# HaydenFaulkner/VidDet

Hardware: AMD Instinct MI355X
Metric: frames/sec (416x416) yolo3_darknet53 fwd+bwd (higher is better)
Workload: dtype f32; 1 GPU; yolo3_darknet53_coco training, batch 64/GPU, 416x416, fp32, fwd+bwd+SGD-momentum (BASELINE configs[2]; the reference trains with SGD, not Adam); classes=80, global_batch=64, parallelism=dp1, hip_graph=False

## Files before the change

### include/viddet_hip.h

```cpp
#ifndef VIDDET_HIP_H
#define VIDDET_HIP_H

#include <stdint.h>

#ifdef __cplusplus
extern "C" {
#endif

#define VD_OK            0
#define VD_EINVAL       -1
#define VD_ELAUNCH      -2
#define VD_EWORKSPACE   -3

#define VD_MAX_TAPS 27

#define VD_EPI_AFFINE    1
#define VD_EPI_LEAKY     2
#define VD_EPI_RESIDUAL  4
#define VD_MATH_SPLIT    16
#define VD_MATH_BF16     32

#define VD_MATH_F16X2    64
#define VD_MATH_NOHALO   128
#define VD_STORE_BF16    256
#define VD_WGRAD_HALO    512
#define VD_CONV_STREAMK  1024
#define VD_CONV_PARITY4  2048
#define VD_CONV_SPLITK   4096
#define VD_SK_MAX_WG        2048
#define VD_SK_HEADER_BYTES  32768
#define VD_SK_SPLIT_CNT_OFF   4096
#define VD_SK_SPLIT_MAX_TILES 4096
#define VD_SK_TIMEOUT_TICKS 4000
#define VD_AMAX_SLOTS    32
#define VD_AMAX_STRIDE   64
#define VD_AMAX_FLOATS   (VD_AMAX_SLOTS * VD_AMAX_STRIDE)

const char* vd_last_error(void);
int vd_version(void);
#define VD_ABI_VERSION 8
int vd_abi_version(void);
int64_t vd_sizeof_desc(int which);

// ... 27 lines not shown
    const float* bs_mean;
    const float* bs_invstd;
    float*  bs_part;
    float   bs_slope;
    const float* amax_in;
    const float* amax_w;
    float*  amax_out;
    void*   sk_ws;
    int64_t sk_ws_bytes;
    int32_t par_cin;
    int32_t par_mask;
} vd_conv_desc;

int vd_conv_igemm(const vd_conv_desc* d, void* stream);
int vd_conv_igemm_streamk(const vd_conv_desc* d);
int64_t vd_conv_igemm_streamk_ws_bytes(void);
int vd_conv_igemm_mtiles(const vd_conv_desc* d);

int vd_conv_igemm_bf16(const vd_conv_desc* d, int out_f32, void* stream);
int vd_conv_igemm_bf16_streamk(const vd_conv_desc* d, int out_f32);
int vd_conv_igemm_bf16_mtiles(const vd_conv_desc* d);
int vd_pack_weight_bf16(const float* wp_f32, void* wp_bf16, int Co, int Co_pad, int Ci, int Ci_pad, int T,
                        void* stream);
int vd_stem_im2col_bf16(const float* in, void* col, int N, int H, int W, int nchw, void* stream);

typedef struct {
    const float* in;
    const float* dout;
    float*       dwp;
    int32_t N, Hi, Wi, Ci;
// ... 164 lines not shown
```

### viddet_amd/csrc/vd_conv.hip

```cpp

#include "vd_conv_igemm.h"

int vd_igemm_sk_dispatch(const vd_conv_desc& d, int tile, hipStream_t s);
int vd_igemm_sk_applies(const vd_conv_desc& d, int tile);
int vd_igemm_par_dispatch(const vd_conv_desc& d, int tile, hipStream_t s);
int vd_igemm_par_tile(int tile);
int vd_igemm_par_bm(int tile);

namespace {

int igemm_resolve_tile(const vd_conv_desc& d) {
    int tile = d.tile;
    if (tile <= 0 || tile > 8) {
        if (d.Co <= 32) tile = 7;
        else if (d.Co <= 64) tile = 6;
        else tile = 2;
    }
    return tile;
}

int igemm_tile_bm(int tile) { return (tile == 4 || tile == 5) ? 64 : 128; }

int igemm_split_resolve_tile(const vd_conv_desc& d) {
    int tile = d.tile;
    if (tile <= 0 || tile > 16) tile = d.Co <= 32 ? 9 : (d.Co <= 64 ? 3 : 1);
    return tile;
}
int igemm_split_tile_bm(int tile) { return (tile >= 13 ? 256 : (tile >= 11 ? 128 : ((tile >= 9 || ((tile - 1) & 3) == 0 || ((tile - 1) & 3) == 2) ? 256 : 128))); }

template <bool XF>
int dispatch_igemm_split(const vd_conv_desc& d, hipStream_t s) {
    if (!XF && (d.flags & VD_CONV_STREAMK) && vd_igemm_sk_dispatch(d, igemm_split_resolve_tile(d), s) == 0) return 0;
    switch (igemm_split_resolve_tile(d)) {
        case 1: return launch_igemm<4, 2, 2, 2, XF, true>(d, s);
        case 2: return launch_igemm<4, 2, 1, 2, XF, true>(d, s);
        case 3: return launch_igemm<4, 2, 2, 1, XF, true>(d, s);
        case 4: return launch_igemm<4, 2, 1, 1, XF, true>(d, s);
        case 5: return launch_igemm<4, 2, 2, 2, XF, true, true>(d, s);
        case 6: return launch_igemm<4, 2, 1, 2, XF, true, true>(d, s);
        case 7: return launch_igemm<4, 2, 2, 1, XF, true, true>(d, s);
        case 8: return launch_igemm<4, 2, 1, 1, XF, true, true>(d, s);
        case 9: return launch_igemm<8, 1, 1, 1, XF, true>(d, s);
        case 10: return launch_igemm<8, 1, 1, 1, XF, true, true>(d, s);
        case 11: return launch_igemm<2, 2, 2, 2, XF, true>(d, s);
        case 12: return launch_igemm<2, 2, 2, 2, XF, true, true>(d, s);
        case 13: return launch_igemm<4, 1, 2, 1, XF, true>(d, s);
// ... 561 lines not shown
                   d->Co == 4 * d->par_cin && d->ldo >= d->par_cin && d->ldo % 4 == 0 && (uintptr_t)d->out % 16 == 0 &&
                   (!(d->flags & VD_EPI_RESIDUAL) || (d->ldr % 4 == 0 && (uintptr_t)d->residual % 16 == 0)),
                   "vd_conv_igemm: VD_CONV_PARITY4 geometry (even output, Co = 4 par_cin, aligned rows)");
        VD_REQUIRE(!d->bs_part || (((uintptr_t)d->bs_z | (uintptr_t)d->bs_scale | (uintptr_t)d->bs_shift | (uintptr_t)d->bs_mean |
                                    (uintptr_t)d->bs_invstd) % 16 == 0), "vd_conv_igemm: VD_CONV_PARITY4 bs_* alignment");
        vd_igemm_par_dispatch(*d, vd_igemm_par_tile(d->tile), s);
        VD_CHECK_LAUNCH("vd_conv_igemm/parity4");
        return VD_OK;
    }
    if (d->in_scale) dispatch_igemm<true>(*d, s);
    else dispatch_igemm<false>(*d, s);
    VD_CHECK_LAUNCH("vd_conv_igemm");
    return VD_OK;
}

int vd_conv_igemm_streamk(const vd_conv_desc* d) {
    if (!d || !(d->flags & VD_CONV_STREAMK) || !(d->flags & VD_MATH_F16X2)) return 0;
    return vd_igemm_sk_applies(*d, igemm_split_resolve_tile(*d));
}

int64_t vd_conv_igemm_streamk_ws_bytes(void) {
    return (int64_t)VD_SK_HEADER_BYTES + (int64_t)device_cus() * 256 * 256 * 4;
}

int vd_conv_igemm_mtiles(const vd_conv_desc* d) {
    if (!d) return 0;
    const int64_t M = (int64_t)d->N * d->Hg * d->Wg;
    if (d->flags & VD_CONV_PARITY4)
        return (int)(vd_cdiv(M, vd_igemm_par_bm(vd_igemm_par_tile(d->tile))) * vd_cdiv(d->Co, 128));
    if (d->flags & (VD_MATH_SPLIT | VD_MATH_BF16 | VD_MATH_F16X2)) return (int)vd_cdiv(M, igemm_split_tile_bm(igemm_split_resolve_tile(*d)));
    return (int)vd_cdiv(M, igemm_tile_bm(igemm_resolve_tile(*d)));
}
// ... 132 lines not shown
```

### viddet_amd/csrc/vd_conv_igemm.h

```cpp
#pragma once
#include "vd_common.h"
#include "vd_wgrad_halo.h"
#include <stdlib.h>

namespace {


#ifndef VD_WG_REMAP
#define VD_WG_REMAP 1
#endif
#ifndef VD_KORDER
#define VD_KORDER 1
#endif
#ifndef VD_SETPRIO
#define VD_SETPRIO 1
#endif
#ifndef VD_PROBE
#define VD_PROBE 0
#endif
#ifndef VD_PD
#define VD_PD 3
#endif
#ifndef VD_BNT
#define VD_BNT 0
// ... 96 lines not shown
template <> struct Terms<3> { static constexpr int N = 6; static constexpr int QA[6] = {1, 2, 0, 1, 0, 0}, QB[6] = {1, 0, 2, 0, 1, 0}; };
template <> struct Terms<2> { static constexpr int N = 3; static constexpr int QA[6] = {1, 0, 0, 0, 0, 0}, QB[6] = {0, 1, 0, 0, 0, 0}; };
template <> struct Terms<1> { static constexpr int N = 1; static constexpr int QA[6] = {0, 0, 0, 0, 0, 0}, QB[6] = {0, 0, 0, 0, 0, 0}; };

__device__ __forceinline__ unsigned udiv_rcp(unsigned n, unsigned d, unsigned rcp) {
    unsigned q = d == 1u ? n : __umulhi(n, rcp);
    q -= (q * d > n) ? 1u : 0u;
    return q;
}

struct RowInfo {
    int64_t off;
    unsigned mask;
};

template <int WM, int WN, int TM, int TN, bool XF, bool SP, bool M16 = false, bool BS = false, int NPL = 3, bool HALO = false, bool SK = false,
          bool PAR = false>
__global__ __launch_bounds__(WM * WN * 64, ((!SP && WM * WN == 8) ? 4 : ((SP && WM * WN == 4) ? 2 : 1))) void k_conv_igemm(const vd_conv_desc p, const int64_t zd_in, const int64_t zd_w, const int sk_lds_flag, const int sk_timeout) {
    static_assert(NPL == 3 || ((NPL == 1 || NPL == 2) && SP), "planes");
    static_assert(!SK || (NPL == 2 && VD_KORDER && !VD_KROT && !XF), "stream-K: the fp16-split tiles, taps-innermost K order");
    static_assert(!PAR || (NPL == 2 && !HALO && !SK && VD_KORDER && !VD_KROT), "parity-fused data gradient: fp16-split tiles, generic loop");
    static_assert(NPL != 2 || !XF, "the fp16 split needs the max-abs of the operand it splits: no in-load transform");
    static_assert(!HALO || (NPL == 2 && WM * WN == 8 && WN * TN * 32 >= 64), "the halo loop exists for the 8-wave fp16-split tiles");
    constexpr int SP_ROWB = NPL * 64;
    constexpr int NTERM = Terms<NPL>::N;
    static_assert(!M16 || SP, "the 16x16x32 shape exists for the bf16 operands of the split arithmetic");
    constexpr int BM = WM * TM * 32, BN = WN * TN * 32;
    constexpr int NT = WM * WN * 64;
    constexpr int RPP = NT / 8;
    constexpr bool BHALF = BN < RPP;
    constexpr int AP = BM / RPP, BP = BHALF ? 1 : BN / RPP;
    static_assert(WM * WN == 4 || WM * WN == 8, "4 or 8 waves");
    static_assert(BM % RPP == 0 && (BHALF || BN % RPP == 0), "tile vs loader");
    static_assert(!BHALF || SP, "the half-populated weight pass exists for the split-math tiles");
    extern __shared__ __attribute__((aligned(16))) float smem[];
    float* As = smem;
    float* Bs = smem + 2 * BM * LDS_LD;
    char* As3 = reinterpret_cast<char*>(smem);
    char* Bs3 = As3 + 2 * BM * SP_ROWB;

    const int64_t M = (int64_t)p.N * p.Hg * p.Wg;
    const int ntile = (p.Co + BN - 1) / BN;
    const int Ktot = p.T * p.Ci;
    constexpr int KU = HALO ? 9 : 1;
    const int upt = p.T * (p.Ci / BK) / KU;
    int sk_nitems = 1, sk_t0 = 0, sk_nwhole = 0, sk_brem = 0, sk_erem = 0, sk_tlast = 0, sk_tfirst = 0, sk_me = 0;
    if (SK) {
        const int G = (int)gridDim.x, g = blockIdx.x & 7, j = blockIdx.x >> 3;
        const int gq = G >> 3, gr = G & 7;
        const int gs = gq + (g < gr ? 1 : 0);
        const int gbase = g * gq + (g < gr ? g : gr);
        const int64_t ntiles_all = vd_cdiv(M, BM) * ntile;
        const int tq = (int)(ntiles_all >> 3), tr = (int)(ntiles_all & 7);
        const int tg0 = g * tq + (g < tr ? g : tr), tgn = tq + (g < tr ? 1 : 0);
// ... 34 lines not shown
    const int lrow = tid >> 3;
    const int lc4 = (tid & 7) * 4;
    int lid = SK ? 0 : vd_xcd_remap(blockIdx.x, gridDim.x);
    int kb = 0, ke = upt;
    int sk_mode = 0;
    if (SK) {
        __syncthreads();
        const bool hasA = sk_erem != 0;
        if (hasA && sk_it == 0) { lid = sk_tlast; ke = sk_erem; sk_mode = 1; }
        else if (sk_it - (hasA ? 1 : 0) < sk_nwhole) lid = sk_t0 + sk_it - (hasA ? 1 : 0);
        else { lid = sk_tfirst; kb = sk_brem; sk_mode = 2; }
    }
    const int mt_all = (int)vd_cdiv(M, BM);
    const int tile_n = SK ? lid / mt_all : lid % ntile, tile_m = SK ? lid % mt_all : lid / ntile;
    RowInfo ri[AP];
    {
        int riy[AP], rix[AP], rfz[AP];
#pragma unroll
        for (int i = 0; i < AP; ++i) {
            const int64_t m = (int64_t)tile_m * BM + lrow + RPP * i;
            const unsigned mu = m < M ? (unsigned)m : 0u;
            const unsigned t = udiv_rcp(mu, (unsigned)p.Wg, rcp_w);
            const int gx = (int)(mu - t * (unsigned)p.Wg);
            const unsigned n_ = udiv_rcp(t, (unsigned)p.Hg, rcp_h);
            const int gy = (int)(t - n_ * (unsigned)p.Hg);
            const int n = (int)n_;
            riy[i] = gy * p.in_stride;
            rix[i] = gx * p.in_stride;
            rfz[i] = p.Kfr == 1 ? 0 : n % p.Kfr;
            ri[i].off = (int64_t)((n * p.Hi + riy[i]) * p.Wi + rix[i]) * p.Ci + lc4;
            ri[i].mask = 0u;
// ... 57 lines not shown
#pragma unroll
                    for (int ni = 0; ni < TN; ++ni)
#pragma unroll
                        for (int q = 0; q < 4; ++q) {
                            const f32x4 v = slot[((mi * TN + ni) * 4 + q) * NT + tid];
#pragma unroll
                            for (int e = 0; e < 4; ++e) acc[mi][ni][4 * q + e] = v[e];
                        }
            } else {
                kb = 0;
                sk_mode = 0;
            }
        }
    }

    constexpr int PD = (VD_PD > 2 && ((WM * WN == 4 && TM * TN == 4) || (M16 && TM * TN == 4))) ? 2 : VD_PD;
    f32x4 ra[PD][AP], rb[PD][BP];
    int t_tap = 0, c0 = VD_KROT ? (int)((unsigned)tile_m % (unsigned)(p.Ci / BK)) * BK : 0;
    if (SK && !HALO) {
        c0 = (kb / p.T) * BK;
        t_tap = kb - (kb / p.T) * p.T;
    }

    const int64_t tap_eo = (int64_t)((tap_dz * p.Hi + tap_dy) * p.Wi + tap_dx) * p.Ci;
    const int tap_eo_lo = (int)(tap_eo & 0xffffffffll), tap_eo_hi = (int)(tap_eo >> 32);
    auto tap_off = [&](int t) -> int64_t {
        const unsigned lo = (unsigned)__builtin_amdgcn_readlane(tap_eo_lo, t);
        const int hi = __builtin_amdgcn_readlane(tap_eo_hi, t);
        return ((int64_t)hi << 32) | (int64_t)lo;
    };
    int64_t tap_soff = tap_off(t_tap);
    auto gload = [&](f32x4 (&ra)[AP], f32x4 (&rb)[BP]) {
        const int64_t soff = tap_soff + c0;
        f32x4 sc = {0.f, 0.f, 0.f, 0.f}, sh = {0.f, 0.f, 0.f, 0.f};
        if (XF) {
            sc = *reinterpret_cast<const f32x4*>(p.in_scale + c0 + lc4);
            sh = *reinterpret_cast<const f32x4*>(p.in_shift + c0 + lc4);
        }
#pragma unroll
        for (int i = 0; i < AP; ++i) {
            const bool ok = (ri[i].mask >> t_tap) & 1u;
            const int64_t o = ri[i].off + soff;
            const int64_t sel = (ok && !(VD_PROBE & 8) && !((VD_PROBE & 32) && t_tap != 0)) ? o : zd_in;
            f32x4 v = *reinterpret_cast<const f32x4*>(p.in + sel);
            if (XF) {
#pragma unroll
                for (int e = 0; e < 4; ++e) {
// ... 430 lines not shown
                }
            }
            if (!late) hstores(u, do_store);
            __syncthreads();
        };
        int ks = 0;
        for (; ks + UNH + PD + 1 <= nks; ks += UNH) {
#pragma unroll
            for (int u = 0; u < UNH; ++u) hstep(u, true, true, true);
        }
        for (; ks < nks; ks += UNH) {
#pragma unroll
            for (int u = 0; u < UNH; ++u)
                if (ks + u < nks) hstep(u, ks + u + 1 < nks, ks + u + PD + 1 < nks, ks + u + 2 < nks);
        }
    } else {
    gload(ra[0], rb[0]);
    STAMP(2);
    lstore(0, ra[0], rb[0]);
    __syncthreads();
    STAMP(3);
    constexpr bool ld = !(VD_PROBE & 1), st = !(VD_PROBE & 2), bar = !(VD_PROBE & 4);
    constexpr int UN = (PD % 2 == 0) ? PD : 2 * PD;
    constexpr bool STAGGER = SP && (WM * WN == 8);
    const bool stag = (wave >> 2) & 1;
#pragma unroll
    for (int d = 1; d < PD; ++d)
        if (d < nks && ld) gload(ra[d], rb[d]);
    int ks = 0;
    if (nks >= PD) {
// ... 43 lines not shown
            __syncthreads();
            if (tid == 0)
                __hip_atomic_fetch_add(reinterpret_cast<unsigned*>(p.sk_ws) + sk_me, 1u, __ATOMIC_RELAXED, __HIP_MEMORY_SCOPE_AGENT);
            continue;
        }
    }
    if (NPL == 2) {
        const int de = -(sexp_a + sexp_b);
#pragma unroll
        for (int mi = 0; mi < TM; ++mi)
#pragma unroll
            for (int ni = 0; ni < TN; ++ni)
#pragma unroll
                for (int r = 0; r < 16; ++r) acc[mi][ni][r] = __builtin_ldexpf(acc[mi][ni][r], de);
    }
    const bool direct = (p.out_stride == 1 && p.out_oy == 0 && p.out_ox == 0 && p.Ho == p.Hg &&
                         p.Wo == p.Wg);
    float* stg = smem + wave * (32 * LDS_LD);
    const int erow = lane >> 3, ec4 = (lane & 7) * 4;
    const bool bstat = BS && p.bs_part != nullptr;
    float bs1[TN][4], bs2[TN][4];
#pragma unroll
    for (int ni = 0; ni < TN; ++ni)
#pragma unroll
        for (int e = 0; e < 4; ++e) bs1[ni][e] = bs2[ni][e] = 0.f;
    const bool vec_ok = (p.ldo % 4 == 0) && ((uintptr_t)p.out % 16 == 0) &&
                        (!(p.flags & VD_EPI_RESIDUAL) || ((p.ldr % 4 == 0) && ((uintptr_t)p.residual % 16 == 0)));
    const bool has_aff = p.flags & VD_EPI_AFFINE, has_leaky = p.flags & VD_EPI_LEAKY, has_res = p.flags & VD_EPI_RESIDUAL;
    bool fast = vec_ok && (p.Co % 4 == 0) && (!has_aff || (((uintptr_t)p.scale | (uintptr_t)p.shift) % 16 == 0));
    if (BS) fast = fast && (!bstat || (((uintptr_t)p.bs_z | (uintptr_t)p.bs_scale | (uintptr_t)p.bs_shift |
                                        (uintptr_t)p.bs_mean | (uintptr_t)p.bs_invstd) % 16 == 0));
    if (SK || fast) {
        constexpr int NB = TM * TN;
        f32x4 sc[TN], sh[TN], qsc[BS ? TN : 1], qsh[BS ? TN : 1], qmu[BS ? TN : 1], qis[BS ? TN : 1];
        int colv[TN];
        const f32x4 ones = {1.f, 1.f, 1.f, 1.f}, zeros = {0.f, 0.f, 0.f, 0.f};
#pragma unroll
        for (int ni = 0; ni < TN; ++ni) {
            const int col = tile_n * BN + wn * TN * 32 + ni * 32 + ec4;
            const int chn = PAR ? col % p.par_cin : col;
            colv[ni] = col < p.Co ? chn : -1;
            const int cc = col < p.Co ? chn : 0;
            sc[ni] = (has_aff && p.scale) ? *reinterpret_cast<const f32x4*>(p.scale + cc) : ones;
            sh[ni] = (has_aff && p.shift) ? *reinterpret_cast<const f32x4*>(p.shift + cc) : zeros;
            if (BS) {
                qsc[ni] = bstat ? *reinterpret_cast<const f32x4*>(p.bs_scale + cc) : zeros;
                qsh[ni] = bstat ? *reinterpret_cast<const f32x4*>(p.bs_shift + cc) : zeros;
// ... 63 lines not shown
                    amx = fmaxf(amx, fmaxf(fmaxf(fabsf(t[0]), fabsf(t[1])), fmaxf(fabsf(t[2]), fabsf(t[3]))));
                }
                if (BS && bstat) {
                    const f32x4 z = rz[BS ? (b & S1) : 0][i];
#pragma unroll
                    for (int e = 0; e < 4; ++e) {
                        const float u = z[e] * qsc[ni][e] + qsh[ni][e];
                        float g = u > 0.f ? t[e] : t[e] * p.bs_slope;
                        g = ok ? g : 0.f;
                        bs1[ni][e] += g;
                        bs2[ni][e] += g * (z[e] - qmu[ni][e]) * qis[ni][e];
                    }
                }
            }
        }
    } else if constexpr (!SK) {
#pragma unroll
    for (int ni = 0; ni < TN; ++ni) {
        const int col = tile_n * BN + wn * TN * 32 + ni * 32 + ec4;
        const int nvalid = p.Co - col;
        float sc[4] = {1.f, 1.f, 1.f, 1.f}, sh[4] = {0.f, 0.f, 0.f, 0.f};
        if (p.flags & VD_EPI_AFFINE) {
#pragma unroll
            for (int e = 0; e < 4; ++e)
                if (e < nvalid) {
                    if (p.scale) sc[e] = p.scale[col + e];
                    if (p.shift) sh[e] = p.shift[col + e];
                }
        }
        float qsc[4], qsh[4], qmu[4], qis[4];
        if (bstat) {
// ... 196 lines not shown
    }
    if (p.amax_out) vd_amax_publish(p.amax_out, amx);
    STAMP(6);
}

const float* zero_page() {
    static const float* zp = nullptr;
    if (!zp) {
        void* q = nullptr;
        if (hipGetSymbolAddress(&q, HIP_SYMBOL(g_zero_page)) != hipSuccess) q = nullptr;
        zp = (const float*)q;
    }
    return zp;
}

template <int WM, int WN, int TM, int TN, bool XF, bool SP, bool M16, bool BS, int NPL, bool HALO = false, bool SK = false, bool PAR = false>
int launch_igemm_bs(const vd_conv_desc& d, hipStream_t s);

inline int64_t halo_lds_bytes(int BM, int BN, int W) { return 2ll * (BM + 2 * (W + 1) + 2) * 128 + 3ll * BN * 128; }

inline bool halo_ok(const vd_conv_desc& d, int BM, int BN) {
    if (!(d.flags & VD_MATH_F16X2) || (d.flags & VD_MATH_NOHALO) || d.in_scale || d.T != 9 || d.in_stride != 1 || d.Kfr != 1 ||
        d.Hg != d.Hi || d.Wg != d.Wi || BN < 64)
        return false;
    for (int t = 0; t < 9; ++t)
        if (d.dy[t] < -1 || d.dy[t] > 1 || d.dx[t] < -1 || d.dx[t] > 1 || d.dz[t] != 0) return false;
    return BM + 2 * (d.Wi + 1) <= 8 * 64 && halo_lds_bytes(BM, BN, d.Wi) <= 160 * 1024;
}

template <int WM, int WN, int TM, int TN, bool XF, bool SP = false, bool M16 = false>
int launch_igemm(const vd_conv_desc& d, hipStream_t s) {
    if (SP && (d.flags & VD_MATH_BF16)) {
        if (d.bs_part) return launch_igemm_bs<WM, WN, TM, TN, false, SP, M16, true, SP ? 1 : 3>(d, s);
        return launch_igemm_bs<WM, WN, TM, TN, false, SP, M16, false, SP ? 1 : 3>(d, s);
    }
    if (SP && (d.flags & VD_MATH_F16X2)) {
        constexpr bool HT_ = SP && WM * WN == 8 && WN * TN * 32 >= 64;
        if (HT_ && halo_ok(d, WM * TM * 32, WN * TN * 32)) {
            if (d.bs_part) return launch_igemm_bs<WM, WN, TM, TN, false, SP, M16, true, SP ? 2 : 3, HT_>(d, s);
            return launch_igemm_bs<WM, WN, TM, TN, false, SP, M16, false, SP ? 2 : 3, HT_>(d, s);
        }
        if (d.bs_part) return launch_igemm_bs<WM, WN, TM, TN, false, SP, M16, true, SP ? 2 : 3>(d, s);
// ... 16 lines not shown
inline int streamk_grid(const vd_conv_desc& d, int BM, int BN, int wg_per_cu) {
    if (!(d.flags & VD_CONV_STREAMK) || !d.sk_ws) return 0;
    auto al16 = [](const void* q) { return (uintptr_t)q % 16 == 0; };
    if (d.ldo % 4 || d.Co % 4 || !al16(d.out) || ((d.flags & VD_EPI_RESIDUAL) && (d.ldr % 4 || !al16(d.residual))) ||
        ((d.flags & VD_EPI_AFFINE) && (!al16(d.scale) || !al16(d.shift))) ||
        (d.bs_part && !(al16(d.bs_z) && al16(d.bs_scale) && al16(d.bs_shift) && al16(d.bs_mean) && al16(d.bs_invstd))))
        return 0;
    const int64_t ntiles = vd_cdiv((int64_t)d.N * d.Hg * d.Wg, BM) * vd_cdiv(d.Co, BN);
    const int G = device_cus() * wg_per_cu;
    if (G > VD_SK_MAX_WG - 2 || G < 8 || (ntiles >> 3) < (G + 7) / 8) return 0;
    if (ntiles <= G + G / 16) return 0;
    if (d.sk_ws_bytes < (int64_t)VD_SK_HEADER_BYTES + (int64_t)G * BM * BN * 4) return 0;
    return G;
}

template <int WM, int WN, int TM, int TN, bool XF, bool SP, bool M16, bool BS, int NPL, bool HALO, bool SK, bool PAR>
int launch_igemm_bs(const vd_conv_desc& d, hipStream_t s) {
    constexpr int BM = WM * TM * 32, BN = WN * TN * 32;
    constexpr int lds0 = SP ? 2 * (BM + BN) * NPL * 64 : 2 * (BM + BN) * LDS_LD * (int)sizeof(float);
    constexpr int lds_epi = WM * WN * 32 * LDS_LD * 4 > WM * BN * 2 * 4 ? WM * WN * 32 * LDS_LD * 4 : WM * BN * 2 * 4;
    constexpr int lds_fixed = lds0 > lds_epi ? lds0 : lds_epi;
    static_assert(lds_fixed + (SK ? 16 : 0) <= 160 * 1024, "LDS budget");
    int lds = lds_fixed;
    if (HALO) {
        const int64_t hb = halo_lds_bytes(BM, BN, d.Wi);
        lds = hb > lds_epi ? (int)hb : lds_epi;
    }
    int64_t nblk = vd_cdiv((int64_t)d.N * d.Hg * d.Wg, BM) * vd_cdiv(d.Co, BN);
    int sk_flag_off = 0;
    if (SK) {
        const int G = streamk_grid(d, BM, BN, (SP && WM * WN == 4) ? 2 : 1);
        lds = (lds + 15) & ~15;
        if (G == 0 || lds + 16 > 160 * 1024) return 1;
        sk_flag_off = lds;
        lds += 16;
        nblk = G;
    }
    static bool attr_done = false;
    auto kfn = k_conv_igemm<WM, WN, TM, TN, XF, SP, M16, BS, NPL, HALO, SK, PAR>;
    if (!attr_done) {
        (void)hipFuncSetAttribute(reinterpret_cast<const void*>(kfn), hipFuncAttributeMaxDynamicSharedMemorySize,
                                  HALO ? 160 * 1024 : lds_fixed + (SK ? 16 : 0));
        attr_done = true;
    }
    const float* zp = zero_page();
    const int64_t zd_in = zp - d.in, zd_w = zp - d.wp;
    static const int sk_timeout = getenv("VD_SK_TIMEOUT_TICKS") ? atoi(getenv("VD_SK_TIMEOUT_TICKS")) : VD_SK_TIMEOUT_TICKS;
    hipLaunchKernelGGL(kfn, dim3((unsigned)nblk), dim3(WM * WN * 64), lds, s, d, zd_in, zd_w, sk_flag_off, sk_timeout);
    return 0;
}

}
```

### viddet_amd/lib.py

```python
import ctypes as C
import os

_HERE = os.path.dirname(os.path.abspath(__file__))
LIB_PATH = os.environ.get("VD_LIB") or os.path.join(_HERE, "csrc", "libviddet_hip.so")

ABI_VERSION = 8
VD_MAX_TAPS = 27
EPI_AFFINE, EPI_LEAKY, EPI_RESIDUAL = 1, 2, 4
MATH_SPLIT = 16
MATH_BF16 = 32
MATH_F16X2 = 64
MATH_NOHALO = 128
STORE_BF16 = 256
WGRAD_HALO = 512
CONV_STREAMK = 1024
CONV_SPLITK = 4096
CONV_PARITY4 = 2048
SK_HEADER_BYTES = 32768
AMAX_SLOTS, AMAX_STRIDE = 32, 64
AMAX_FLOATS = AMAX_SLOTS * AMAX_STRIDE

_fp = C.c_void_p


class ConvDesc(C.Structure):
    _fields_ = [
        ("in_", _fp), ("wp", _fp), ("out", _fp), ("scale", _fp), ("shift", _fp), ("residual", _fp),
        ("N", C.c_int32), ("Hi", C.c_int32), ("Wi", C.c_int32), ("Ci", C.c_int32),
        ("Hg", C.c_int32), ("Wg", C.c_int32), ("in_stride", C.c_int32), ("T", C.c_int32),
        ("dy", C.c_int32 * VD_MAX_TAPS), ("dx", C.c_int32 * VD_MAX_TAPS), ("dz", C.c_int32 * VD_MAX_TAPS),
        ("Kfr", C.c_int32),
# ... 32 lines not shown
        ("head", _fp * 3), ("g", C.c_int32 * 3), ("ldh", C.c_int32),
        ("stride", C.c_float * 3), ("anchors", (C.c_float * 6) * 3),
        ("B", C.c_int32), ("C", C.c_int32),
    ]


_i, _i64, _f, _d, _p = C.c_int, C.c_int64, C.c_float, C.c_double, C.c_void_p
SIGNATURES = {
    "vd_last_error": (C.c_char_p, []),
    "vd_version": (_i, []),
    "vd_abi_version": (_i, []),
    "vd_sizeof_desc": (_i64, [_i]),
    "vd_conv_igemm": (_i, [C.POINTER(ConvDesc), _p]),
    "vd_conv_igemm_mtiles": (_i, [C.POINTER(ConvDesc)]),
    "vd_conv_igemm_streamk": (_i, [C.POINTER(ConvDesc)]),
    "vd_conv_igemm_streamk_ws_bytes": (_i64, []),
    "vd_conv_igemm_bf16": (_i, [C.POINTER(ConvDesc), _i, _p]),
    "vd_conv_igemm_bf16_mtiles": (_i, [C.POINTER(ConvDesc)]),
    "vd_conv_igemm_bf16_streamk": (_i, [C.POINTER(ConvDesc), _i]),
    "vd_pack_weight_bf16": (_i, [_p, _p, _i, _i, _i, _i, _i, _p]),
    "vd_stem_im2col_bf16": (_i, [_p, _p, _i, _i, _i, _i, _p]),
    "vd_conv_wgrad_ws_bytes": (_i64, [C.POINTER(WgradDesc)]),
    "vd_conv_wgrad": (_i, [C.POINTER(WgradDesc), _p, _i64, _p]),
    "vd_conv_wgrad_uses_halo": (_i, [C.POINTER(WgradDesc)]),
    "vd_stem_im2col": (_i, [_p, _p, _i, _i, _i, _i, _p]),
    "vd_pack_weight_fwd": (_i, [_p, _p, _i, _i, _i, _i, _i, _i, _p]),
    "vd_pack_weight_dgrad": (_i, [_p, _p, _i, _i, _i, _i, _i, _i, C.POINTER(C.c_int32), _i, _i, _p]),
    "vd_pack_weight_dgrad_s2": (_i, [_p, _p, _i, _i, _i, C.POINTER(C.c_int32), _p]),
    "vd_unpack_wgrad": (_i, [_p, _p, _i, _i, _i, _i, _i, _p]),
    "vd_bn_stats_ws_bytes": (_i64, [_i64, _i]),
# ... 107 lines not shown
```

### viddet_amd/model.py

```python
import ctypes as C
import math
import re
from collections import OrderedDict

import numpy as np
import torch

from . import lib as L
from . import ops
from .lib import ConvDesc, WgradDesc, EPI_AFFINE, EPI_LEAKY, EPI_RESIDUAL
from .ops import round_up, fwd_taps, dgrad_plans

from .consts import ANCHORS, STRIDES, BN_EPS, BN_MOMENTUM, LEAKY_SLOPE


class Slot:

    def __init__(self):
        self.value = None


class Program:

    def __init__(self):
# ... 38 lines not shown
        for (fname, fn, args), meta in zip(self.recs, self.meta):
            if fname is None:
                if meta and meta.get('kind') == 'collective':
                    fn()
                continue
            a = [x.value if isinstance(x, Slot) else x for x in args]
            if fname in select:
                e0, e1 = torch.cuda.Event(enable_timing=True), torch.cuda.Event(enable_timing=True)
                e0.record()
                rc = fn(*a, s)
                e1.record()
                if fname in ("vd_conv_igemm", "vd_conv_wgrad"):
                    d = args[0]._obj
                    meta = dict(meta or {}, split=bool(d.flags & L.MATH_SPLIT), bf16=bool(d.flags & L.MATH_BF16),
                                f16x2=bool(d.flags & L.MATH_F16X2), nohalo=bool(d.flags & L.MATH_NOHALO), tile=int(getattr(d, "tile", 0)),
                                streamk=bool(fname == "vd_conv_igemm" and L.load().vd_conv_igemm_streamk(args[0])))
                    if fname == "vd_conv_wgrad":
                        meta["wgrad_halo"] = bool(L.load().vd_conv_wgrad_uses_halo(args[0]))
                    if fname == "vd_conv_igemm" and meta.get("bytes"):
                        out_bytes = 4.0 * d.N * d.Hg * d.Wg * d.Co
                        extra = (out_bytes if d.residual else 0.0) + (out_bytes if getattr(d, "bs_part", None) else 0.0)
                        meta["bytes_epilogue_reads"] = extra
                        meta["bytes"] = meta["bytes"] + extra
                if fname == "vd_conv_igemm_bf16":
                    form = int(L.load().vd_conv_igemm_bf16_streamk(args[0], args[1]))
                    meta = dict(meta or {}, tile=int(args[0]._obj.tile), nohalo=bool(args[0]._obj.flags & L.MATH_NOHALO),
                                streamk=form == 1, splitk=form == 2)
                out.append((fname, meta, e0, e1))
            else:
                rc = fn(*a, s)
            if rc != 0:
                L.check(rc, fname)
        return out


class TuneCache(dict):

    def __init__(self):
        super().__init__()
        self._loaded, self._dirty, self.tuned, self.hits, self._synced_world = False, False, 0, 0, 1

    @staticmethod
    def library_id():
        import hashlib
        import os
        here = os.path.dirname(os.path.abspath(__file__))
        srcs = [os.path.join(here, "csrc", f) for f in ("vd_conv.hip", "vd_conv_igemm.h", "vd_conv_sk.hip", "vd_conv_par.hip",
                                                         "vd_conv_bf16.hip", "vd_conv_igemm_bf16.h", "vd_conv_bf16_sk.hip", "vd_conv_c32_bf16.hip",
                                                         "vd_wgrad_halo.hip", "vd_common.h")]
        h = hashlib.sha256()
        if all(os.path.exists(f) for f in srcs):
            for f in srcs:
                h.update(open(f, "rb").read())
        else:
            h.update(open(L.LIB_PATH, "rb").read())
        for sw in ("VD_WGRAD_RESERVE",):
            if os.environ.get(sw):
                h.update(("%s=%s" % (sw, os.environ[sw])).encode())
        return h.hexdigest()[:12]

    def path(self):
        import os
# ... 19 lines not shown
    def _read_file(self):
        import ast
        import json
        import os
        out = {}
        p = self.path()
        if p is None or not os.path.exists(p):
            return out
        try:
            doc = json.load(open(p))
            if doc.get("library") not in (None, self.library_id()):
                return out
            arch = self.device_arch()
            if arch is not None and doc.get("device") not in (None, arch):
                return out
            for k, v in doc.get("entries", {}).items():
                out[ast.literal_eval(k)] = tuple(v) if isinstance(v, list) else v
        except (OSError, ValueError, SyntaxError) as e:
            print("viddet_amd: ignoring tuning table %s (%s)" % (p, e), flush=True)
            return {}
        return out

    def load(self):
        import os
        self._loaded = True
        world = self._world()
        self._synced_world = world
        if world > 1 and os.environ.get("VD_TUNE_AGREE", "1") != "0":
            box = [self._read_file() if torch.distributed.get_rank() == 0 else None]
            torch.distributed.broadcast_object_list(box, src=0)
# ... 31 lines not shown
        return tuple(box[0]) if isinstance(box[0], list) else box[0]

    def save(self):
        import json
        import os
        if not self._dirty:
            return
        self._dirty = False
        p = self.path()
        if p is None:
            return
        if torch.distributed.is_available() and torch.distributed.is_initialized() and torch.distributed.get_rank() != 0:
            return
        try:
            os.makedirs(os.path.dirname(p) or ".", exist_ok=True)
            doc = {"library": self.library_id(), "device": self.device_arch() or "gfx950",
                   "entries": {repr(k): (list(v) if isinstance(v, tuple) else v) for k, v in sorted(self.items(), key=lambda kv: repr(kv[0]))}}
            tmp = "%s.%d.tmp" % (p, os.getpid())
            with open(tmp, "w") as f:
                json.dump(doc, f, indent=0)
            os.replace(tmp, p)
        except OSError as e:
            print("viddet_amd: could not write tuning table %s (%s)" % (p, e), flush=True)


_TUNE_CACHE = TuneCache()


def _parity_streams():
    return __import__('os').environ.get('VD_PARITY_STREAMS', '1') == '1'


# ... 4 lines not shown
def _bf16_pitch(c):
    return c if (c == 32 or c % 64 == 0) else round_up(c, 64)



def fp32_math():
    import os
    m = _MATH_OVERRIDE[0] or os.environ.get("VD_FP32_MATH", "auto")
    if m not in _MATH_MODES:
        raise ValueError("VD_FP32_MATH must be one of %s, got %r" % ("|".join(_MATH_MODES), m))
    return m


_MATH_OVERRIDE = [None]
_MATH_MODES = ("native", "split", "split2", "auto", "bf16")
_ALL_MATH = L.MATH_SPLIT | L.MATH_BF16 | L.MATH_F16X2 | L.MATH_NOHALO | L.CONV_STREAMK


def _streamk_on():
    return __import__('os').environ.get('VD_STREAMK', '1') != '0'


def _streamk_applies(d, fl, tile):
    if not (d.sk_ws and (fl & L.MATH_F16X2)):
        return False
    keep = (d.flags, d.tile)
    d.flags, d.tile = (d.flags & ~_ALL_MATH) | fl | L.CONV_STREAMK, tile
    try:
        return bool(L.load().vd_conv_igemm_streamk(C.byref(d)))
    finally:
        d.flags, d.tile = keep


def set_conv_math(mode):
    assert mode is None or mode in _MATH_MODES
# ... 28 lines not shown
            cands += [(fl, t) for t in (3, 4, 7, 8)] + ([(fl, t) for t in (15, 16)] if not (fl & L.MATH_F16X2 and not fl & L.MATH_NOHALO and d.T == 9 and d.in_stride == 1 and d.Hg == d.Hi) else [])
        else:
            cands += [(fl, t) for t in (1, 2, 3, 4, 5, 6, 7, 8)] + ([(fl, t) for t in (11, 12)] if not (fl & L.MATH_F16X2 and not fl & L.MATH_NOHALO and d.T == 9 and d.in_stride == 1 and d.Hg == d.Hi) else [])
    return cands


def autotune_desc(d, reps=3):
    import os
    math = fp32_math()
    base = d.flags & ~_ALL_MATH
    if os.environ.get("VD_AUTOTUNE", "1") == "0":
        f16 = L.MATH_F16X2 if (d.amax_in and d.amax_w and not d.in_scale) else L.MATH_SPLIT
        d.flags = base | {"split": L.MATH_SPLIT, "split2": f16, "bf16": L.MATH_BF16}.get(math, 0)
        if d.flags & L.MATH_F16X2 and d.T >= 9 and d.sk_ws and _streamk_on():
            d.flags |= L.CONV_STREAMK
        if os.environ.get("VD_TILE_ALT", "0") == "1":
            alt = [t for fl, t in _tile_candidates(d, math if math != "auto" else "native") if fl == (d.flags & _ALL_MATH)]
            if alt:
                d.tile = alt[-1]
        return
    lib = L.load()
    s = L.stream_ptr()
    key = (math, d.N, d.Hi, d.Wi, d.Ci, d.Hg, d.Wg, d.in_stride, d.T, d.Co, d.out_stride, base, bool(d.in_scale),
           bool(d.stats_part), bool(d.amax_in and d.amax_w), bool(d.amax_out), d.Kfr, bool(d.bs_part))
    if key in _TUNE_CACHE:
        fl, d.tile = _TUNE_CACHE[key]
        d.flags = base | fl
        return
    cands = _tile_candidates(d, math)
    best = cands[0]
    if len(cands) > 1:
        def time_of(fl, c, n):
            d.flags, d.tile = base | fl, c
            L.check(lib.vd_conv_igemm(C.byref(d), s), 'vd_conv_igemm/tune')
            e0, e1 = torch.cuda.Event(enable_timing=True), torch.cuda.Event(enable_timing=True)
            e0.record()
            for _ in range(n):
                lib.vd_conv_igemm(C.byref(d), s)
            e1.record()
            e1.synchronize()
            t = e0.elapsed_time(e1) / n
            if os.environ.get("VD_TUNE_VERBOSE") == "1":
                print("igemm tune %s math %d tile %d: %.4f ms (%d launches)" % (key[1:11], fl, c, t, n), flush=True)
            return t
        ranked = sorted((time_of(fl, c, reps), (fl, c)) for fl, c in cands)
        if _streamk_on():
            sk = [(fl | L.CONV_STREAMK, c) for _, (fl, c) in ranked[:3] if _streamk_applies(d, fl, c)]
            ranked = sorted(ranked + [(time_of(fl, c, reps), (fl, c)) for fl, c in sk])
        best = ranked[0][1]
        close = [fc for t, fc in ranked if t <= 1.04 * ranked[0][0]][:3]
        if len(close) > 1:
            best = min((time_of(fl, c, 3 * reps), (fl, c)) for fl, c in close)[1]
    best = _TUNE_CACHE.agree(tuple(best))
    d.flags, d.tile = base | best[0], best[1]
    _TUNE_CACHE[key] = best


def _wgrad_halo_applies(d, flags):
    keep = d.flags
    d.flags = flags | L.WGRAD_HALO
    try:
        return bool(L.load().vd_conv_wgrad_uses_halo(C.byref(d)))
    finally:
# ... 2378 lines not shown
```

Before: 1045 frames/s.

## Add specialized pointwise (1x1) implicit-GEMM conv path with deeper LDS pipeline

Adds a PW template variant of the fp16-split implicit-GEMM kernel for 1x1 stride-1 convolutions. It computes row offsets as plain m*Ci with no tap or halo geometry, always uses the vectorized direct epilogue, and when LDS allows uses a four-slot double-step pipeline that loads two K-steps per barrier, with wave staggering. The autotuner adds pointwise candidates built from the top-ranked tiles, and the tune cache gains an 'extends' base file. The intent is to cut address arithmetic and barrier overhead for the many 1x1 convs in Darknet53, at the cost of more template instantiations and higher LDS and register use.

```diff
diff --git a/include/viddet_hip.h b/include/viddet_hip.h
--- a/include/viddet_hip.h
+++ b/include/viddet_hip.h
@@ -27,6 +27,7 @@
 #define VD_CONV_STREAMK  1024
 #define VD_CONV_PARITY4  2048
 #define VD_CONV_SPLITK   4096
+#define VD_CONV_POINTWISE 8192
 #define VD_SK_MAX_WG        2048
 #define VD_SK_HEADER_BYTES  32768
 #define VD_SK_SPLIT_CNT_OFF   4096
@@ -84,6 +85,7 @@
 
 int vd_conv_igemm(const vd_conv_desc* d, void* stream);
 int vd_conv_igemm_streamk(const vd_conv_desc* d);
+int vd_conv_igemm_pointwise(const vd_conv_desc* d);
 int64_t vd_conv_igemm_streamk_ws_bytes(void);
 int vd_conv_igemm_mtiles(const vd_conv_desc* d);
 
diff --git a/viddet_amd/csrc/vd_conv.hip b/viddet_amd/csrc/vd_conv.hip
--- a/viddet_amd/csrc/vd_conv.hip
+++ b/viddet_amd/csrc/vd_conv.hip
@@ -3,6 +3,8 @@
 
 int vd_igemm_sk_dispatch(const vd_conv_desc& d, int tile, hipStream_t s);
 int vd_igemm_sk_applies(const vd_conv_desc& d, int tile);
+int vd_igemm_pw_dispatch(const vd_conv_desc& d, int tile, hipStream_t s);
+int vd_igemm_pw_applies(const vd_conv_desc& d, int tile);
 int vd_igemm_par_dispatch(const vd_conv_desc& d, int tile, hipStream_t s);
 int vd_igemm_par_tile(int tile);
 int vd_igemm_par_bm(int tile);
@@ -30,6 +32,7 @@
 
 template <bool XF>
 int dispatch_igemm_split(const vd_conv_desc& d, hipStream_t s) {
+    if (!XF && (d.flags & VD_CONV_POINTWISE) && vd_igemm_pw_dispatch(d, igemm_split_resolve_tile(d), s) == 0) return 0;
     if (!XF && (d.flags & VD_CONV_STREAMK) && vd_igemm_sk_dispatch(d, igemm_split_resolve_tile(d), s) == 0) return 0;
     switch (igemm_split_resolve_tile(d)) {
         case 1: return launch_igemm<4, 2, 2, 2, XF, true>(d, s);
@@ -621,8 +624,14 @@
     return VD_OK;
 }
 
+int vd_conv_igemm_pointwise(const vd_conv_desc* d) {
+    if (!d || !(d->flags & VD_CONV_POINTWISE) || !(d->flags & VD_MATH_F16X2)) return 0;
+    return vd_igemm_pw_applies(*d, igemm_split_resolve_tile(*d));
+}
+
 int vd_conv_igemm_streamk(const vd_conv_desc* d) {
     if (!d || !(d->flags & VD_CONV_STREAMK) || !(d->flags & VD_MATH_F16X2)) return 0;
+    if (vd_conv_igemm_pointwise(d)) return 0;
     return vd_igemm_sk_applies(*d, igemm_split_resolve_tile(*d));
 }
 
diff --git a/viddet_amd/csrc/vd_conv_igemm.h b/viddet_amd/csrc/vd_conv_igemm.h
--- a/viddet_amd/csrc/vd_conv_igemm.h
+++ b/viddet_amd/csrc/vd_conv_igemm.h
@@ -134,14 +134,17 @@
     unsigned mask;
 };
 
+constexpr bool pw_two_steps(int BM, int BN, int waves) { return 4 * (BM + BN) * 128 <= (waves == 8 ? 160 : 80) * 1024; }
+
 template <int WM, int WN, int TM, int TN, bool XF, bool SP, bool M16 = false, bool BS = false, int NPL = 3, bool HALO = false, bool SK = false,
-          bool PAR = false>
+          bool PAR = false, bool PW = false>
 __global__ __launch_bounds__(WM * WN * 64, ((!SP && WM * WN == 8) ? 4 : ((SP && WM * WN == 4) ? 2 : 1))) void k_conv_igemm(const vd_conv_desc p, const int64_t zd_in, const int64_t zd_w, const int sk_lds_flag, const int sk_timeout) {
     static_assert(NPL == 3 || ((NPL == 1 || NPL == 2) && SP), "planes");
     static_assert(!SK || (NPL == 2 && VD_KORDER && !VD_KROT && !XF), "stream-K: the fp16-split tiles, taps-innermost K order");
     static_assert(!PAR || (NPL == 2 && !HALO && !SK && VD_KORDER && !VD_KROT), "parity-fused data gradient: fp16-split tiles, generic loop");
     static_assert(NPL != 2 || !XF, "the fp16 split needs the max-abs of the operand it splits: no in-load transform");
     static_assert(!HALO || (NPL == 2 && WM * WN == 8 && WN * TN * 32 >= 64), "the halo loop exists for the 8-wave fp16-split tiles");
+    static_assert(!PW || (NPL == 2 && !HALO && !SK && !PAR && !XF && VD_KORDER && !VD_KROT), "pointwise form: fp16-split tiles, generic loop");
     constexpr int SP_ROWB = NPL * 64;
     constexpr int NTERM = Terms<NPL>::N;
     static_assert(!M16 || SP, "the 16x16x32 shape exists for the bf16 operands of the split arithmetic");
@@ -157,7 +160,9 @@
     float* As = smem;
     float* Bs = smem + 2 * BM * LDS_LD;
     char* As3 = reinterpret_cast<char*>(smem);
-    char* Bs3 = As3 + 2 * BM * SP_ROWB;
+    constexpr bool PW2 = PW && pw_two_steps(BM, BN, WM * WN);
+    constexpr int NSLOT = PW2 ? 4 : 2;
+    char* Bs3 = As3 + NSLOT * BM * SP_ROWB;
 
     const int64_t M = (int64_t)p.N * p.Hg * p.Wg;
     const int ntile = (p.Co + BN - 1) / BN;
@@ -222,7 +227,14 @@
     const int mt_all = (int)vd_cdiv(M, BM);
     const int tile_n = SK ? lid / mt_all : lid % ntile, tile_m = SK ? lid % mt_all : lid / ntile;
     RowInfo ri[AP];
-    {
+    if constexpr (PW) {
+#pragma unroll
+        for (int i = 0; i < AP; ++i) {
+            const int64_t m = (int64_t)tile_m * BM + lrow + RPP * i;
+            ri[i].off = m * p.Ci + lc4;
+            ri[i].mask = m < M ? 1u : 0u;
+        }
+    } else {
         int riy[AP], rix[AP], rfz[AP];
 #pragma unroll
         for (int i = 0; i < AP; ++i) {
@@ -310,7 +322,7 @@
         }
     }
 
-    constexpr int PD = (VD_PD > 2 && ((WM * WN == 4 && TM * TN == 4) || (M16 && TM * TN == 4))) ? 2 : VD_PD;
+    constexpr int PD = PW2 ? 4 : ((VD_PD > 2 && ((WM * WN == 4 && TM * TN == 4) || (M16 && TM * TN == 4))) ? 2 : VD_PD);
     f32x4 ra[PD][AP], rb[PD][BP];
     int t_tap = 0, c0 = VD_KROT ? (int)((unsigned)tile_m % (unsigned)(p.Ci / BK)) * BK : 0;
     if (SK && !HALO) {
@@ -327,6 +339,21 @@
     };
     int64_t tap_soff = tap_off(t_tap);
     auto gload = [&](f32x4 (&ra)[AP], f32x4 (&rb)[BP]) {
+        if constexpr (PW) {
+            const bool inr = c0 < p.Ci;
+#pragma unroll
+            for (int i = 0; i < AP; ++i) {
+                const int64_t sel = (ri[i].mask && inr) ? ri[i].off + c0 : zd_in;
+                ra[i] = *reinterpret_cast<const f32x4*>(p.in + sel);
+            }
+#pragma unroll
+            for (int i = 0; i < BP; ++i) {
+                const int64_t sel = (boff[i] >= 0 && inr) ? boff[i] + c0 : zd_w;
+                rb[i] = *reinterpret_cast<const f32x4*>(p.wp + sel);
+            }
+            c0 += BK;
+            return;
+        }
         const int64_t soff = tap_soff + c0;
         f32x4 sc = {0.f, 0.f, 0.f, 0.f}, sh = {0.f, 0.f, 0.f, 0.f};
         if (XF) {
@@ -787,6 +814,41 @@
             for (int u = 0; u < UNH; ++u)
                 if (ks + u < nks) hstep(u, ks + u + 1 < nks, ks + u + PD + 1 < nks, ks + u + 2 < nks);
         }
+    } else if constexpr (PW2) {
+        const bool stag = (WM * WN == 8) && ((wave >> 2) & 1);
+        const int nst = (nks + 1) >> 1;
+#pragma unroll
+        for (int d = 0; d < 4; ++d) gload(ra[d], rb[d]);
+        lstore(0, ra[0], rb[0]);
+        lstore(1, ra[1], rb[1]);
+        __syncthreads();
+        auto stage = [&](int b, bool more, bool two) {
+            if (more) {
+                gload(ra[b], rb[b]);
+                gload(ra[b + 1], rb[b + 1]);
+            }
+            if (stag) {
+                if (more) lstore((b + 2) & 3, ra[(b + 2) & 3], rb[(b + 2) & 3]);
+                compute(b);
+                if (more) lstore((b + 3) & 3, ra[(b + 3) & 3], rb[(b + 3) & 3]);
+                if (two) compute(b + 1);
+            } else {
+                compute(b);
+                if (more) lstore((b + 2) & 3, ra[(b + 2) & 3], rb[(b + 2) & 3]);
+                if (two) compute(b + 1);
+                if (more) lstore((b + 3) & 3, ra[(b + 3) & 3], rb[(b + 3) & 3]);
+            }
+            __syncthreads();
+        };
+        int st = 0;
+        for (; st + 2 < nst; st += 2) {
+            stage(0, true, true);
+            stage(2, true, true);
+        }
+        for (; st < nst; st += 2) {
+            stage(0, st + 1 < nst, 2 * st + 1 < nks);
+            if (st + 1 < nst) stage(2, false, 2 * st + 3 < nks);
+        }
     } else {
     gload(ra[0], rb[0]);
     STAMP(2);
@@ -860,8 +922,8 @@
 #pragma unroll
                 for (int r = 0; r < 16; ++r) acc[mi][ni][r] = __builtin_ldexpf(acc[mi][ni][r], de);
     }
-    const bool direct = (p.out_stride == 1 && p.out_oy == 0 && p.out_ox == 0 && p.Ho == p.Hg &&
-                         p.Wo == p.Wg);
+    const bool direct = PW || (p.out_stride == 1 && p.out_oy == 0 && p.out_ox == 0 && p.Ho == p.Hg &&
+                                p.Wo == p.Wg);
     float* stg = smem + wave * (32 * LDS_LD);
     const int erow = lane >> 3, ec4 = (lane & 7) * 4;
     const bool bstat = BS && p.bs_part != nullptr;
@@ -876,7 +938,7 @@
     bool fast = vec_ok && (p.Co % 4 == 0) && (!has_aff || (((uintptr_t)p.scale | (uintptr_t)p.shift) % 16 == 0));
     if (BS) fast = fast && (!bstat || (((uintptr_t)p.bs_z | (uintptr_t)p.bs_scale | (uintptr_t)p.bs_shift |
                                         (uintptr_t)p.bs_mean | (uintptr_t)p.bs_invstd) % 16 == 0));
-    if (SK || fast) {
+    if (SK || PW || fast) {
         constexpr int NB = TM * TN;
         f32x4 sc[TN], sh[TN], qsc[BS ? TN : 1], qsh[BS ? TN : 1], qmu[BS ? TN : 1], qis[BS ? TN : 1];
         int colv[TN];
@@ -970,7 +1032,7 @@
                 }
             }
         }
-    } else if constexpr (!SK) {
+    } else if constexpr (!SK && !PW) {
 #pragma unroll
     for (int ni = 0; ni < TN; ++ni) {
         const int col = tile_n * BN + wn * TN * 32 + ni * 32 + ec4;
@@ -1197,7 +1259,8 @@
     return zp;
 }
 
-template <int WM, int WN, int TM, int TN, bool XF, bool SP, bool M16, bool BS, int NPL, bool HALO = false, bool SK = false, bool PAR = false>
+template <int WM, int WN, int TM, int TN, bool XF, bool SP, bool M16, bool BS, int NPL, bool HALO = false, bool SK = false, bool PAR = false,
+          bool PW = false>
 int launch_igemm_bs(const vd_conv_desc& d, hipStream_t s);
 
 inline int64_t halo_lds_bytes(int BM, int BN, int W) { return 2ll * (BM + 2 * (W + 1) + 2) * 128 + 3ll * BN * 128; }
@@ -1209,6 +1272,18 @@
     for (int t = 0; t < 9; ++t)
         if (d.dy[t] < -1 || d.dy[t] > 1 || d.dx[t] < -1 || d.dx[t] > 1 || d.dz[t] != 0) return false;
     return BM + 2 * (d.Wi + 1) <= 8 * 64 && halo_lds_bytes(BM, BN, d.Wi) <= 160 * 1024;
+}
+
+inline bool pw_ok(const vd_conv_desc& d) {
+    if (!(d.flags & VD_MATH_F16X2) || (d.flags & VD_CONV_PARITY4) || d.in_scale || d.T != 1 || d.dy[0] || d.dx[0] || d.dz[0] ||
+        d.in_stride != 1 || d.Hg != d.Hi || d.Wg != d.Wi || d.out_stride != 1 || d.out_oy || d.out_ox || d.Ho != d.Hg || d.Wo != d.Wg)
+        return false;
+    auto al16 = [](const void* q) { return (uintptr_t)q % 16 == 0; };
+    if (d.ldo % 4 || d.Co % 4 || !al16(d.out) || ((d.flags & VD_EPI_RESIDUAL) && (d.ldr % 4 || !al16(d.residual))) ||
+        ((d.flags & VD_EPI_AFFINE) && (!al16(d.scale) || !al16(d.shift))) ||
+        (d.bs_part && !(al16(d.bs_z) && al16(d.bs_scale) && al16(d.bs_shift) && al16(d.bs_mean) && al16(d.bs_invstd))))
+        return false;
+    return true;
 }
 
 template <int WM, int WN, int TM, int TN, bool XF, bool SP = false, bool M16 = false>
@@ -1255,10 +1330,10 @@
     return G;
 }
 
-template <int WM, int WN, int TM, int TN, bool XF, bool SP, bool M16, bool BS, int NPL, bool HALO, bool SK, bool PAR>
+template <int WM, int WN, int TM, int TN, bool XF, bool SP, bool M16, bool BS, int NPL, bool HALO, bool SK, bool PAR, bool PW>
 int launch_igemm_bs(const vd_conv_desc& d, hipStream_t s) {
     constexpr int BM = WM * TM * 32, BN = WN * TN * 32;
-    constexpr int lds0 = SP ? 2 * (BM + BN) * NPL * 64 : 2 * (BM + BN) * LDS_LD * (int)sizeof(float);
+    constexpr int lds0 = SP ? ((PW && pw_two_steps(BM, BN, WM * WN)) ? 4 : 2) * (BM + BN) * NPL * 64 : 2 * (BM + BN) * LDS_LD * (int)sizeof(float);
     constexpr int lds_epi = WM * WN * 32 * LDS_LD * 4 > WM * BN * 2 * 4 ? WM * WN * 32 * LDS_LD * 4 : WM * BN * 2 * 4;
     constexpr int lds_fixed = lds0 > lds_epi ? lds0 : lds_epi;
     static_assert(lds_fixed + (SK ? 16 : 0) <= 160 * 1024, "LDS budget");
@@ -1278,7 +1353,7 @@
         nblk = G;
     }
     static bool attr_done = false;
-    auto kfn = k_conv_igemm<WM, WN, TM, TN, XF, SP, M16, BS, NPL, HALO, SK, PAR>;
+    auto kfn = k_conv_igemm<WM, WN, TM, TN, XF, SP, M16, BS, NPL, HALO, SK, PAR, PW>;
     if (!attr_done) {
         (void)hipFuncSetAttribute(reinterpret_cast<const void*>(kfn), hipFuncAttributeMaxDynamicSharedMemorySize,
                                   HALO ? 160 * 1024 : lds_fixed + (SK ? 16 : 0));
diff --git a/viddet_amd/csrc/vd_conv_pw.hip b/viddet_amd/csrc/vd_conv_pw.hip
--- /dev/null
+++ b/viddet_amd/csrc/vd_conv_pw.hip
@@ -0,0 +1,36 @@
+#include "vd_conv_igemm.h"
+
+namespace {
+
+template <int WM, int WN, int TM, int TN, bool M16>
+int launch_pw(const vd_conv_desc& d, hipStream_t s) {
+    if (d.bs_part) return launch_igemm_bs<WM, WN, TM, TN, false, true, M16, true, 2, false, false, false, true>(d, s);
+    return launch_igemm_bs<WM, WN, TM, TN, false, true, M16, false, 2, false, false, false, true>(d, s);
+}
+
+}
+
+int vd_igemm_pw_applies(const vd_conv_desc& d, int tile) { return (tile >= 1 && tile <= 16 && pw_ok(d)) ? 1 : 0; }
+
+int vd_igemm_pw_dispatch(const vd_conv_desc& d, int tile, hipStream_t s) {
+    if (!pw_ok(d)) return 1;
+    switch (tile) {
+        case 1: return launch_pw<4, 2, 2, 2, false>(d, s);
+        case 2: return launch_pw<4, 2, 1, 2, false>(d, s);
+        case 3: return launch_pw<4, 2, 2, 1, false>(d, s);
+        case 4: return launch_pw<4, 2, 1, 1, false>(d, s);
+        case 5: return launch_pw<4, 2, 2, 2, true>(d, s);
+        case 6: return launch_pw<4, 2, 1, 2, true>(d, s);
+        case 7: return launch_pw<4, 2, 2, 1, true>(d, s);
+        case 8: return launch_pw<4, 2, 1, 1, true>(d, s);
+        case 9: return launch_pw<8, 1, 1, 1, false>(d, s);
+        case 10: return launch_pw<8, 1, 1, 1, true>(d, s);
+        case 11: return launch_pw<2, 2, 2, 2, false>(d, s);
+        case 12: return launch_pw<2, 2, 2, 2, true>(d, s);
+        case 13: return launch_pw<4, 1, 2, 1, false>(d, s);
+        case 14: return launch_pw<4, 1, 2, 1, true>(d, s);
+        case 15: return launch_pw<4, 1, 2, 2, false>(d, s);
+        case 16: return launch_pw<4, 1, 2, 2, true>(d, s);
+        default: return 1;
+    }
+}
diff --git a/viddet_amd/lib.py b/viddet_amd/lib.py
--- a/viddet_amd/lib.py
+++ b/viddet_amd/lib.py
@@ -15,6 +15,7 @@
 WGRAD_HALO = 512
 CONV_STREAMK = 1024
 CONV_SPLITK = 4096
+CONV_POINTWISE = 8192
 CONV_PARITY4 = 2048
 SK_HEADER_BYTES = 32768
 AMAX_SLOTS, AMAX_STRIDE = 32, 64
@@ -77,6 +78,7 @@
     "vd_conv_igemm": (_i, [C.POINTER(ConvDesc), _p]),
     "vd_conv_igemm_mtiles": (_i, [C.POINTER(ConvDesc)]),
     "vd_conv_igemm_streamk": (_i, [C.POINTER(ConvDesc)]),
+    "vd_conv_igemm_pointwise": (_i, [C.POINTER(ConvDesc)]),
     "vd_conv_igemm_streamk_ws_bytes": (_i64, []),
     "vd_conv_igemm_bf16": (_i, [C.POINTER(ConvDesc), _i, _p]),
     "vd_conv_igemm_bf16_mtiles": (_i, [C.POINTER(ConvDesc)]),
diff --git a/viddet_amd/model.py b/viddet_amd/model.py
--- a/viddet_amd/model.py
+++ b/viddet_amd/model.py
@@ -76,7 +76,8 @@
                     d = args[0]._obj
                     meta = dict(meta or {}, split=bool(d.flags & L.MATH_SPLIT), bf16=bool(d.flags & L.MATH_BF16),
                                 f16x2=bool(d.flags & L.MATH_F16X2), nohalo=bool(d.flags & L.MATH_NOHALO), tile=int(getattr(d, "tile", 0)),
-                                streamk=bool(fname == "vd_conv_igemm" and L.load().vd_conv_igemm_streamk(args[0])))
+                                streamk=bool(fname == "vd_conv_igemm" and L.load().vd_conv_igemm_streamk(args[0])),
+                                pointwise=bool(fname == "vd_conv_igemm" and L.load().vd_conv_igemm_pointwise(args[0])))
                     if fname == "vd_conv_wgrad":
                         meta["wgrad_halo"] = bool(L.load().vd_conv_wgrad_uses_halo(args[0]))
                     if fname == "vd_conv_igemm" and meta.get("bytes"):
@@ -101,13 +102,14 @@
     def __init__(self):
         super().__init__()
         self._loaded, self._dirty, self.tuned, self.hits, self._synced_world = False, False, 0, 0, 1
+        self._extends, self._base = None, {}
 
     @staticmethod
     def library_id():
         import hashlib
         import os
         here = os.path.dirname(os.path.abspath(__file__))
-        srcs = [os.path.join(here, "csrc", f) for f in ("vd_conv.hip", "vd_conv_igemm.h", "vd_conv_sk.hip", "vd_conv_par.hip",
+        srcs = [os.path.join(here, "csrc", f) for f in ("vd_conv.hip", "vd_conv_igemm.h", "vd_conv_sk.hip", "vd_conv_pw.hip", "vd_conv_par.hip",
                                                          "vd_conv_bf16.hip", "vd_conv_igemm_bf16.h", "vd_conv_bf16_sk.hip", "vd_conv_c32_bf16.hip",
                                                          "vd_wgrad_halo.hip", "vd_common.h")]
         h = hashlib.sha256()
@@ -157,6 +159,13 @@
             arch = self.device_arch()
             if arch is not None and doc.get("device") not in (None, arch):
                 return out
+            ext = doc.get("extends")
+            if ext:
+                bdoc = json.load(open(os.path.join(os.path.dirname(p), os.path.basename(ext))))
+                if arch is None or bdoc.get("device") in (None, arch):
+                    for k, v in bdoc.get("entries", {}).items():
+                        out[ast.literal_eval(k)] = tuple(v) if isinstance(v, list) else v
+                self._extends, self._base = os.path.basename(ext), dict(out)
             for k, v in doc.get("entries", {}).items():
                 out[ast.literal_eval(k)] = tuple(v) if isinstance(v, list) else v
         except (OSError, ValueError, SyntaxError) as e:
@@ -218,8 +227,11 @@
             return
         try:
             os.makedirs(os.path.dirname(p) or ".", exist_ok=True)
+            own = [(k, v) for k, v in self.items() if not (k in self._base and self._base[k] == v)]
             doc = {"library": self.library_id(), "device": self.device_arch() or "gfx950",
-                   "entries": {repr(k): (list(v) if isinstance(v, tuple) else v) for k, v in sorted(self.items(), key=lambda kv: repr(kv[0]))}}
+                   "entries": {repr(k): (list(v) if isinstance(v, tuple) else v) for k, v in sorted(own, key=lambda kv: repr(kv[0]))}}
+            if self._extends:
+                doc["extends"] = self._extends
             tmp = "%s.%d.tmp" % (p, os.getpid())
             with open(tmp, "w") as f:
                 json.dump(doc, f, indent=0)
@@ -254,11 +266,26 @@
 
 _MATH_OVERRIDE = [None]
 _MATH_MODES = ("native", "split", "split2", "auto", "bf16")
-_ALL_MATH = L.MATH_SPLIT | L.MATH_BF16 | L.MATH_F16X2 | L.MATH_NOHALO | L.CONV_STREAMK
+_ALL_MATH = L.MATH_SPLIT | L.MATH_BF16 | L.MATH_F16X2 | L.MATH_NOHALO | L.CONV_STREAMK | L.CONV_POINTWISE
 
 
 def _streamk_on():
     return __import__('os').environ.get('VD_STREAMK', '1') != '0'
+
+
+def _pointwise_on():
+    return __import__('os').environ.get('VD_POINTWISE', '1') != '0'
+
+
+def _pointwise_applies(d, fl, tile):
+    if not (fl & L.MATH_F16X2) or d.T != 1:
+        return False
+    keep = (d.flags, d.tile)
+    d.flags, d.tile = (d.flags & ~_ALL_MATH) | fl | L.CONV_POINTWISE, tile
+    try:
+        return bool(L.load().vd_conv_igemm_pointwise(C.byref(d)))
+    finally:
+        d.flags, d.tile = keep
 
 
 def _streamk_applies(d, fl, tile):
@@ -317,6 +344,8 @@
         d.flags = base | {"split": L.MATH_SPLIT, "split2": f16, "bf16": L.MATH_BF16}.get(math, 0)
         if d.flags & L.MATH_F16X2 and d.T >= 9 and d.sk_ws and _streamk_on():
             d.flags |= L.CONV_STREAMK
+        if d.flags & L.MATH_F16X2 and d.T == 1 and _pointwise_on():
+            d.flags |= L.CONV_POINTWISE
         if os.environ.get("VD_TILE_ALT", "0") == "1":
             alt = [t for fl, t in _tile_candidates(d, math if math != "auto" else "native") if fl == (d.flags & _ALL_MATH)]
             if alt:
@@ -328,6 +357,8 @@
            bool(d.stats_part), bool(d.amax_in and d.amax_w), bool(d.amax_out), d.Kfr, bool(d.bs_part))
     if key in _TUNE_CACHE:
         fl, d.tile = _TUNE_CACHE[key]
+        if not _pointwise_on():
+            fl &= ~L.CONV_POINTWISE
         d.flags = base | fl
         return
     cands = _tile_candidates(d, math)
@@ -350,6 +381,9 @@
         if _streamk_on():
             sk = [(fl | L.CONV_STREAMK, c) for _, (fl, c) in ranked[:3] if _streamk_applies(d, fl, c)]
             ranked = sorted(ranked + [(time_of(fl, c, reps), (fl, c)) for fl, c in sk])
+        if _pointwise_on():
+            pw = [(fl | L.CONV_POINTWISE, c) for _, (fl, c) in ranked[:4] if not (fl & L.CONV_STREAMK) and _pointwise_applies(d, fl, c)]
+            ranked = sorted(ranked + [(time_of(fl, c, reps), (fl, c)) for fl, c in pw])
         best = ranked[0][1]
         close = [fc for t, fc in ranked if t <= 1.04 * ranked[0][0]][:3]
         if len(close) > 1:
```

New measurement: 1044 frames/s. No clear change (-0.1%).
